# GadGadGad/Convolutional-KAN-for-Image-Classification

Hardware: AMD Instinct MI355X
Metric: images/sec fwd+bwd KAN-VGG11 3x32x32 bs=256/GPU (higher is better)
Workload: dtype f32

## Files before the change

### convolutional-kan-for-image-classification_amd/_lib.py

```python
from __future__ import annotations

import ctypes as C
import os
from typing import Optional

_HERE = os.path.dirname(os.path.abspath(__file__))
LIB_PATH = os.environ.get("KANCONV_LIB") or os.path.join(_HERE, "libkanconv.so")

KAN_MAX_PLANES = 16
KAN_MAX_TABLE = 32
KAN_FP_WORDS = 192
BASIS_BSPLINE, BASIS_RBF, BASIS_CHEBY, BASIS_POLY, BASIS_FOURIER, BASIS_RELU, BASIS_GRAM = 0, 1, 2, 3, 4, 5, 6
ACT_NONE, ACT_IDENTITY, ACT_GELU, ACT_SILU, ACT_RELU, ACT_TANH, ACT_SIGMOID, ACT_GELU_TANH = -1, 0, 1, 2, 3, 4, 5, 6


class KanGeom(C.Structure):
    _fields_ = [(n, C.c_int) for n in ("B", "C", "H", "W", "O", "Ho", "Wo", "kh", "kw", "sh", "sw", "ph", "pw", "dh", "dw", "groups")] + \
               [("x_bstride", C.c_longlong), ("y_bstride", C.c_longlong)]


class KanBasis(C.Structure):
    _fields_ = [("kind", C.c_int), ("n_basis", C.c_int), ("order", C.c_int), ("act", C.c_int),
                ("p0", C.c_float), ("p1", C.c_float), ("table", C.c_float * KAN_MAX_TABLE), ("chan_table", C.c_void_p)]


class KanPlan(C.Structure):
    _fields_ = [(n, C.c_int) for n in ("P", "K", "IPC", "KC", "Kpad", "Opad", "fwd_splits", "bwd_data_splits", "bwd_weight_splits",
                                          "fwd_target", "bwd_data_target", "bwd_weight_target", "x_pm_wanted", "dz_pm_wanted", "bwd_weight_expanded", "row_blocks", "e_pm_wanted", "fwd_expanded", "fwd_halo", "bwd_weight_halo",
                                          "fwd_band", "bwd_weight_band")] + \
               [(n, C.c_longlong) for n in ("packed_weight_bytes", "bwd_data_weight_bytes", "fwd_slab_elems", "bwd_data_slab_elems",
                                            "bwd_weight_slab_elems", "e_pm_elems")]


class KanWavGeom(C.Structure):
    _fields_ = [(n, C.c_int) for n in ("B", "C", "H", "W", "O", "Ho", "Wo", "kh", "kw", "sh", "sw", "ph", "pw", "dh", "dw", "wavelet")] + \
               [("x_bstride", C.c_longlong), ("u_bstride", C.c_longlong)]


WAVELETS = {"mexican_hat": 0, "morlet": 1, "dog": 2, "meyer": 3, "shannon": 4}

_P, _I, _LL, _F, _D = C.c_void_p, C.c_int, C.c_longlong, C.c_float, C.c_double
_GP, _BP = C.POINTER(KanGeom), C.POINTER(KanBasis)
SIGNATURES = {
    "kan_version": (C.c_char_p, []),
    "kan_last_error": (C.c_char_p, []),
    "kan_plan": (_I, [_GP, _BP, C.POINTER(KanPlan)]),
    "kan_pack_weights": (_I, [_P, _P, _P, _P, _GP, _BP, _P]),
    "kan_pack_cacheable": (_I, [_GP, _BP]),
    "kan_pack_weights_cached": (_I, [_P, _P, _P, _P, _GP, _BP, _P, _I, _I, _I, _P]),
    "kan_conv_fwd": (_I, [_P, _P, _P, _P, _GP, _BP, _P, _P]),
    "kan_position_major": (_I, [_P, _P, _I, _I, _I, _LL, _P]),
    "kan_conv_bwd_data": (_I, [_P, _P, _P, _P, _P, _P, _GP, _BP, _P, _P]),
    "kan_conv_bwd_data_params": (_I, [_P, _P, _P, _P, _P, _P, _P, _GP, _BP, _P, _P]),
    "kan_conv_bwd_weight": (_I, [_P, _P, _P, _P, _GP, _BP, _P, _P, _P]),
    "kan_position_major_expanded": (_I, [_P, _P, _GP, _BP, _P]),
    "kan_conv_fwd_expanded": (_I, [_P, _P, _P, _GP, _BP, _P]),
    "kan_conv_bwd_weight_expanded": (_I, [_P, _P, _P, _GP, _BP, _P]),
    "kan_unpack_wgrad": (_I, [_P, _P, _P, _GP, _BP, _P]),
    "kan_slab_reduce": (_I, [_P, _I, _LL, _P, _I, _I, _I, _LL, _P]),
    "kan_instnorm_prelu_fwd": (_I, [_P, _I, _LL, _P, _P, _P, _P, _P, _P, _P, _I, _I, _I, _LL, _F, _I, _P]),
    "kan_instnorm_prelu_bwd": (_I, [_P, _P, _P, _P, _P, _P, _P, _P, _P, _P, _P, _I, _I, _I, _LL, _I, _P]),
    "kan_instnorm_prelu_pool_fwd": (_I, [_P, _I, _LL, _P, _P, _P, _P, _P, _P, _P, _P, _I, _I, _I, _I, _LL, _F, _I, _P]),
    "kan_instnorm_prelu_pool_bwd": (_I, [_P, _P, _P, _P, _P, _P, _P, _P, _P, _P, _P, _P, _I, _I, _I, _I, _LL, _I, _P]),
    "kan_instnorm_prelu_poolk_fwd": (_I, [_P, _I, _LL, _P, _P, _P, _P, _P, _P, _P, _P, _I, _I, _I, _I, _LL, _F, _I, _I, _I, _P]),
    "kan_instnorm_prelu_poolk_bwd": (_I, [_P, _P, _P, _P, _P, _P, _P, _P, _P, _P, _P, _P, _I, _I, _I, _I, _LL, _I, _I, _I, _P]),
    "kan_split_supported": (_I, [C.POINTER(KanGeom), C.POINTER(KanBasis)]),
    "kan_split_weight_bytes": (_LL, [C.POINTER(KanGeom), C.POINTER(KanBasis)]),
    "kan_split_pack_weights": (_I, [_P, _P, _P, C.POINTER(KanGeom), C.POINTER(KanBasis), _P]),
    "kan_conv_fwd_split": (_I, [_P, _P, _P, C.POINTER(KanGeom), C.POINTER(KanBasis), _P]),
# ... 39 lines not shown
```

### convolutional-kan-for-image-classification_amd/csrc/kan_internal.h

```cpp
#pragma once
#include <type_traits>
#include "kanconv.h"

int kan_fail_msg(const char* fmt, const char* a);
int kan_raise_lds_limit(const void* kernel, int bytes);

enum : int {
    FAST_GENERIC = 0,
    FAST_BSPLINE_SILU = 1,
    FAST_BSPLINE_GELU = 2,
    FAST_RBF8 = 3,
    FAST_CHEBY5 = 4,
    FAST_CHEBY4 = 5,
    FAST_POLY4 = 6,
    FAST_POLY3 = 7,
    FAST_RBF5 = 8,
    FAST_RELU8 = 9,
    FAST_GRAM4 = 10,
    FAST_POLY1 = 11,
    FAST_LAST = 11
};
enum : unsigned {
    ON_TAP_MAJOR = 1u << 0,
    ON_BIG_TILES = 1u << 1,
    ON_HALO_FWD = 1u << 2,
    ON_HALO_BWD_WEIGHT = 1u << 3,
    ON_BAND_FWD = 1u << 4,
    ON_BAND_BWD_WEIGHT = 1u << 5,
    ON_EXPANDED_FWD = 1u << 6,
    ON_EXPANDED = 1u << 7,
    ON_ROWBLK_BWD_DATA = 1u << 8,
};
struct FastSpec {
    int kind, planes;
    bool base;
    bool xn_fwd, xn_bwd;
    int kc;
    unsigned routes;
};
constexpr FastSpec fast_spec(int f) {
    constexpr unsigned bspline = ON_TAP_MAJOR | ON_BIG_TILES | ON_HALO_FWD | ON_HALO_BWD_WEIGHT | ON_BAND_FWD | ON_BAND_BWD_WEIGHT |
                                 ON_EXPANDED_FWD | ON_EXPANDED | ON_ROWBLK_BWD_DATA;
    switch (f) {
        case FAST_BSPLINE_SILU: case FAST_BSPLINE_GELU: return {KAN_BASIS_BSPLINE, 9, true, false, false, 18, bspline};
        case FAST_RBF8: return {KAN_BASIS_RBF, 9, true, true, true, 18, ON_TAP_MAJOR | ON_BAND_FWD | ON_BAND_BWD_WEIGHT};
        case FAST_RBF5: return {KAN_BASIS_RBF, 6, true, true, true, 18, ON_TAP_MAJOR};
        case FAST_CHEBY5: return {KAN_BASIS_CHEBY, 5, false, false, false, 16, ON_TAP_MAJOR | ON_BIG_TILES | ON_BAND_FWD | ON_BAND_BWD_WEIGHT};
        case FAST_CHEBY4: return {KAN_BASIS_CHEBY, 4, false, false, false, 16, ON_TAP_MAJOR | ON_HALO_FWD | ON_BAND_FWD};
        case FAST_POLY4: return {KAN_BASIS_POLY, 5, true, true, false, 16, ON_TAP_MAJOR | ON_BIG_TILES | ON_HALO_FWD | ON_BAND_FWD};
        case FAST_POLY3: return {KAN_BASIS_POLY, 4, true, true, false, 16, ON_TAP_MAJOR};
        case FAST_POLY1: return {KAN_BASIS_POLY, 2, true, true, false, 16, ON_TAP_MAJOR};
        case FAST_RELU8: return {KAN_BASIS_RELU, 9, true, false, false, 16, ON_HALO_FWD | ON_HALO_BWD_WEIGHT | ON_EXPANDED_FWD | ON_EXPANDED};
        case FAST_GRAM4: return {KAN_BASIS_GRAM, 5, true, false, false, 16, ON_HALO_FWD | ON_HALO_BWD_WEIGHT | ON_EXPANDED};
        default: return {-1, 0, false, true, true, 0, 0};
    }
}
constexpr int fast_kind(int f) { return fast_spec(f).kind; }
constexpr int fast_planes(int f) { return fast_spec(f).planes; }
constexpr bool fast_has(int f, unsigned routes) { return (fast_spec(f).routes & routes) == routes && f != FAST_GENERIC; }

template <int V> using IC = std::integral_constant<int, V>;
template <unsigned ROUTES, int F = 1, class Fn>
bool dispatch_fast(int f, Fn&& fn) {
    if constexpr (F > FAST_LAST) {
        return false;
// ... 28 lines not shown
    int cells;
    int slots;
    int TS;
    int lds_bytes, wgs_per_cu;
    int fwd_splits;
    int bw_ok, bw_WR, bw_NI, bw_NT, bw_tiles_o, bw_row_tiles, bw_TPI, bw_ptiles, bw_cells, bw_slots, bw_lds_bytes, bw_splits;
    unsigned short bw_ph_rt0[KAN_BAND_MAX_PHASES + 1];
    unsigned char ph_a[KAN_BAND_MAX_PHASES], ph_b[KAN_BAND_MAX_PHASES];
    short ph_tap0[KAN_BAND_MAX_PHASES + 1];
    unsigned short tap_shift[KAN_BAND_MAX_TAPS];
    unsigned short tap_rt[KAN_BAND_MAX_TAPS];
    short tap_step[KAN_BAND_MAX_TAPS], tap_nt[KAN_BAND_MAX_TAPS];
} KanBandCfg;

void kan_band_cfg(const KanGeom* g, const KanBasis* b, int fast, KanBandCfg* cfg);
int kan_band_bwd_weight_launch(const float* dz, const float* x, const float* xn, float* dwp, const KanGeom* g, const KanBasis* b,
                               const KanBandCfg* cfg, int splits, long long slab_elems, void* stream);
int kan_band_fwd_launch(const float* x, const float* xn, const float* wp, float* z, const KanGeom* g, const KanBasis* b,
                        const KanBandCfg* cfg, int splits, long long slab_elems, void* stream);

constexpr int DW_T = 9;
constexpr int DW_MAX_TP = 96;

enum class Route { TAP_MAJOR, DW, BAND, HALO, EXPANDED };

struct FwdCfg { int TO, TP, tiles_o, tiles_p, chunks, splits, slots; };
struct BdCfg { int CH, tiles_c, tiles_p, n_ob, Opad32, chunks, splits; };
struct BwCfg { int TR, TO, tiles_r, tiles_o, chunks, splits, slots; };
struct BwHaloCfg { int R, nimg, spb, n_bands, tiles_r, tiles_o, splits, bands_per_split; };

struct ConvPlan {
    KanPlan pub;
    int fast;
    Route fwd, bwd_data, bwd_weight;
    bool pm_fwd, pm_bwd_data, pm_bwd_weight;
    bool rowblk_bwd_data;
    bool pmdma_xcd, pm_lpt, pm_xcd;
    FwdCfg fc;
    BdCfg bd;
    BwCfg bw;
    BwHaloCfg bwh;
    KanBandCfg band;
};
int plan_conv(const KanGeom* g, const KanBasis* b, ConvPlan* cp);

int live_taps_out(const KanGeom* g, int hw);
int live_taps_in(const KanGeom* g, int hw);
// ... 3 lines not shown
```

### convolutional-kan-for-image-classification_amd/csrc/kan_plan.hip

```cpp
#include <hip/hip_runtime.h>
#include <cstdio>
#include <cstdlib>
#include <cstring>
#include "kanconv.h"
#include "kan_device.h"
#include "kan_common.h"
#include "kan_internal.h"

namespace {

int fail(const char* msg) { return kan_fail_msg("%s", msg); }

int check(const KanGeom* g, const KanBasis* b) {
    if (!g || !b) return fail("null geometry/basis");
    if (g->groups < 0 || g->groups > 65535) return fail("groups out of range");
    if (g->B <= 0 || g->C <= 0 || g->O <= 0 || g->H <= 0 || g->W <= 0 || g->Ho <= 0 || g->Wo <= 0) return fail("non-positive dimension");
    if (g->kh <= 0 || g->kw <= 0 || g->sh <= 0 || g->sw <= 0 || g->dh <= 0 || g->dw <= 0 || g->ph < 0 || g->pw < 0) return fail("bad conv parameters");
    if (g->kh > 255 || g->kw > 255 || g->C > 65535) return fail("kernel size / channel count out of supported range");
    if ((g->H + 2 * g->ph - g->dh * (g->kh - 1) - 1) / g->sh + 1 != g->Ho || (g->W + 2 * g->pw - g->dw * (g->kw - 1) - 1) / g->sw + 1 != g->Wo)
        return fail("Ho/Wo inconsistent with H/W, kernel, stride, padding, dilation");
    if ((long long)g->B * g->Ho * g->Wo >= (1ll << 31) || (long long)g->B * g->H * g->W >= (1ll << 31)) return fail("pixel count exceeds int32");
    if ((long long)g->B * g->x_bstride * 4 >= (1ll << 31) || (long long)g->B * g->y_bstride * 4 >= (1ll << 31))
        return fail("activation tensors must be smaller than 2 GiB (32-bit buffer offsets)");
    if (g->x_bstride < (long long)ngroups(g) * g->C * g->H * g->W || g->y_bstride < (long long)ngroups(g) * g->O * g->Ho * g->Wo)
// ... 124 lines not shown
    return !tuning_off("KAN_BD_ROWBLK") && fast_has(f, ON_ROWBLK_BWD_DATA) && !pm_bwd_data && g->H == 4 && g->W == 4 && g->Ho == 4 && g->Wo == 4 &&
           g->kh == 3 && g->kw == 3 && g->sh == 1 && g->sw == 1 && g->ph == 1 && g->pw == 1 && g->dh == 1 && g->dw == 1 && g->B % 8 == 0 && g->O % 16 == 0;
}
struct LiveClass { long long tiles; int live_steps; };

int pick_target_steps(const LiveClass* cls, int ncls, int min_steps, double slab_bytes, int* max_splits, long long SLOTS = 1024) {
    int hi = 1;
    for (int i = 0; i < ncls; ++i) if (cls[i].live_steps > hi) hi = cls[i].live_steps;
    int best = hi; double best_cost = -1; int best_ms = 1;
    for (int t = min_steps < hi ? min_steps : hi; t <= hi; ++t) {
        long long wgs = 0; int ms = 1;
        for (int i = 0; i < ncls; ++i) {
            const int sp = cls[i].live_steps > 0 ? ceil_div(cls[i].live_steps, t) : 1;
            wgs += cls[i].tiles * sp;
            if (sp > ms) ms = sp;
        }
        const long long rounds = (wgs + SLOTS - 1) / SLOTS;
        const double cost = (double)(rounds * (t + 6)) + ms * slab_cost_steps(slab_bytes);
        if (best_cost < 0 || cost < best_cost) { best_cost = cost; best = t; best_ms = ms; }
    }
    *max_splits = best_ms;
    return best;
}
BdCfg bd_cfg(const KanGeom* g, const KanPlan& pl) {
    BdCfg c;
    c.CH = 64 / pl.P;
    c.tiles_c = ceil_div(g->C, 2 * c.CH);
    c.tiles_p = ceil_div((long long)g->B * g->H * g->W, 128);
    c.n_ob = ceil_div(g->O, 16);
    c.Opad32 = round_up(g->O, 32);
    c.chunks = g->kh * g->kw * c.n_ob;
    c.splits = pick_splits((long long)c.tiles_c * c.tiles_p * ngroups(g), c.chunks, 8, 4.0 * g->B * g->C * g->H * g->W * ngroups(g));
    return c;
}
bool pmdma_bwd_weight(const KanGeom* g, const KanBasis* b, int f, bool want_pm_bw) {
    if (tuning_off("KAN_PMDMA") || !fast_has(f, ON_EXPANDED)) return false;
    if (!want_pm_bw) return false;
    const int P = b->n_basis + (b->act != KAN_ACT_NONE);
    return (g->C * P) % 128 == 0 && g->B % 16 == 0 && round_up(g->O, 64) % 128 == 0 &&
           (long long)g->C * g->H * g->W * P * g->B * 4 < (1ll << 31);
}
bool halo_bwd_weight(const KanGeom* g, int f, bool pmdma_bw) {
    if (tuning_off("KAN_HALO_BW") || !fast_has(f, ON_HALO_BWD_WEIGHT)) return false;
    if (g->kh != 3 || g->kw != 3 || g->sh != 1 || g->sw != 1 || g->dh != 1 || g->dw != 1 || g->ph != 1 || g->pw != 1) return false;
    if (round_up(g->O, 64) % 128 != 0 || g->C > 65535 / 81) return false;
    if (g->H != g->W) return false;
// ... 102 lines not shown
    if (int rc = check(g, b)) return rc;
    ConvPlan& c = *cp;
    KanPlan* pl = &c.pub;
    const int T = g->kh * g->kw, G = ngroups(g), f = fast_variant(b);
    c.fast = f;
    const bool pm_shape = pmdma_fwd_shape(g, f);
    c.pm_fwd = want_pix_major(g, b, PM_FWD, pm_shape);
    c.pm_bwd_data = want_pix_major(g, b, PM_BWD_DATA, false);
    const bool want_pm_bw = want_pix_major(g, b, PM_BWD_WEIGHT, false);
    const bool dw = dw_direct(g, b);
    const bool halo = halo_fwd(g, b, f, c.pm_fwd);
    c.band.ok = c.band.bw_ok = 0;
    const bool band = band_fwd(g, b, f, dw, c.pm_fwd, halo, &c.band);
    const bool pmdma_fwd = pm_shape && c.pm_fwd;
    const bool pmdma_bw = pmdma_bwd_weight(g, b, f, want_pm_bw);
    const bool halo_bw = halo_bwd_weight(g, f, pmdma_bw);
    c.pm_bwd_weight = want_pm_bw && !halo_bw;
    const bool band_bw = band && c.band.bw_ok && !want_pm_bw && !tuning_off("KAN_BAND_BW");
    c.rowblk_bwd_data = rowblk_bwd_data(g, f, c.pm_bwd_data);
    c.pmdma_xcd = tuning_on("KAN_PMDMA_XCD");
    c.pm_lpt = !tuning_off("KAN_PM_LPT");
    c.pm_xcd = !tuning_off("KAN_PM_XCD");
    c.fwd = dw ? Route::DW : band ? Route::BAND : halo ? Route::HALO : pmdma_fwd ? Route::EXPANDED : Route::TAP_MAJOR;
    c.bwd_data = dw ? Route::DW : Route::TAP_MAJOR;
    c.bwd_weight = dw ? Route::DW : band_bw ? Route::BAND : halo_bw ? Route::HALO : pmdma_bw ? Route::EXPANDED : Route::TAP_MAJOR;
    pl->P = b->n_basis + (b->act != KAN_ACT_NONE);
    pl->K = g->C * T * pl->P;
    {
        int i18 = 18 / pl->P, i16 = 16 / pl->P;
        if (i18 > 4) i18 = 4;
        if (i16 > 4) i16 = 4;
        const bool use18 = (long long)i18 * pl->P * 16 > (long long)i16 * pl->P * 18;
        pl->KC = use18 ? 18 : 16;
        pl->IPC = use18 ? i18 : i16;
        if (pl->P >= 10 && pl->P <= 12) { pl->KC = 12; pl->IPC = 1; }
        if (halo) { pl->KC = 2 * pl->P; pl->IPC = 2; }
    }
    pl->Kpad = ceil_div(g->C * T, pl->IPC) * pl->KC;
    if (band) { pl->KC = c.band.NPLE; pl->IPC = c.band.NG; pl->Kpad = c.band.n_steps * c.band.NPLE; }
    pl->Opad = round_up(g->O, 64);
    pl->packed_weight_bytes = (long long)G * pl->Kpad * pl->Opad * 4;
    c.bd = bd_cfg(g, *pl);
    pl->bwd_data_weight_bytes = (long long)G * T * c.bd.Opad32 * c.bd.tiles_c * 128 * 4;
    pl->fwd_slab_elems = (long long)g->B * g->y_bstride;
    pl->bwd_data_slab_elems = (long long)g->B * g->x_bstride;
    pl->bwd_weight_slab_elems = (long long)G * pl->K * pl->Opad;
    const bool big = big_tiles(f, *pl);
// ... 50 lines not shown
```

### convolutional-kan-for-image-classification_amd/csrc/kanconv.hip

```cpp
#include <hip/hip_runtime.h>
#include <cstdio>
#include <cstdlib>
#include <cstring>
#include <cmath>
#include <cstdint>
#include <mutex>
#include <type_traits>
#include <vector>
#include "kanconv.h"
#include "kan_device.h"

#include "kan_common.h"
#include "kan_internal.h"

namespace {


thread_local char g_err[512] = "";
int fail(const char* fmt, const char* a = "") {
    snprintf(g_err, sizeof(g_err), fmt, a);
    return -1;
}
}
int kan_fail_msg(const char* fmt, const char* a) { return fail(fmt, a); }
// ... 567 lines not shown
    int base = 0;
    int m = M;
#pragma unroll
    for (int off = 32; off >= 1; off >>= 1) {
        if (m > 1) {
            const int h = m / 2;
            const bool up = (lane & off) != 0;
#pragma unroll
            for (int i = 0; i < M / 2; ++i) {
                if (i < h) {
                    const float keep = up ? v[h + i] : v[i], send = up ? v[i] : v[h + i];
                    v[i] = keep + __shfl_xor(send, off, 64);
                }
            }
            base += up ? h : 0;
            m = h;
        } else {
            v[0] += __shfl_xor(v[0], off, 64);
        }
    }
    idx = base; tot = v[0];
}

template <int KIND, int FAST, int RB = 0>
__global__ __launch_bounds__(256, 4) void k_conv_bwd_data(
    const float* __restrict__ dz, const float* __restrict__ x, const float* __restrict__ xn, const float* __restrict__ wd,
    float* __restrict__ dx, float* __restrict__ dxn, DevGeom g, DevBasis bs, int CH, int n_ct, int n_ob, int Opad16,
    int n_chunks, int chunks_per_split, long long slab_elems, unsigned dz_bytes, TilePerm perm, float* __restrict__ dpar) {
    constexpr int TP = 128, KD = 16, NT = 256;
    __shared__ __attribute__((aligned(16))) float smem[2 * 2 * KD * 128];
    __shared__ float sTab[KAN_MAX_TABLE];

    const int tid = threadIdx.x, lane = tid & 63;
    const int wave = __builtin_amdgcn_readfirstlane(tid >> 6);
    const int w_r = wave >> 1, w_p = wave & 1;
    const int HoWo = g.Ho * g.Wo, HW = g.H * g.W, P = bs.P;
    const int Min = g.B * HW;
    const BlockId blk = xcd_block_order(false);
    const int grp = blk.y / n_ct;
    const int px_tile0 = (perm.n ? (int)perm.idx[blk.x] : blk.x) * TP, ct = blk.y - grp * n_ct;
    const int ncol = n_ct * 128;
    const int pxl = (wave & 1) * 64 + lane, ol0 = wave >> 1;
    const bool idle_rows = (ct * 2 + w_r) * CH >= g.C;
    {
        const size_t xo = (size_t)grp * g.C * HW;
        x += xo; xn += xo; dx += xo; if (dxn) dxn += xo;
// ... 135 lines not shown
    };
    int ch = next_live(ch0);
    if (ch < ch1) { if (RB) issue_rb(ch, 0); else issue(ch, 0); }
    const int ar = w_r * 64 + (lane & 31), bp = w_p * 64 + (lane & 31), kh2 = lane >> 5;
    for (int cur = 0; ch < ch1; cur ^= 1) {
        asm volatile("s_waitcnt vmcnt(0)" ::: "memory");
        __syncthreads();
        const bool mixed_now = pend_mixed;
        ch = next_live(ch + 1);
        if (ch < ch1) { if (RB) issue_rb(ch, cur ^ 1); else issue(ch, cur ^ 1); }
        const float* cW = smem + cur * (2 * KD * 128);
        const float* cG = cW + KD * 128;
        const unsigned aw = lds_addr(cW + kh2 * 128 + ar), ag = lds_addr(cG + kh2 * TP + bp);
        if (RB) {
            const bool l0b = !(mixed_now && w_p == 0), l1a = !(mixed_now && w_p == 1);
            if (!idle_rows) KAN_MFMA_STEP_LIVE(KD / 2, aw, 128, ag, TP, true, l0b, l1a, true);
        } else if (!idle_rows) KAN_MFMA_STEP(KD / 2, aw, 128, ag, TP);
    }

    const bool same_in = (x == xn);
    const bool split_out = (dxn != nullptr);
    float* dxs = dx + (size_t)blk.z * slab_elems;
    float* dxns = split_out ? dxn + (size_t)blk.z * slab_elems : nullptr;
#define KAN_G_TO_LDS(half)                                                                                                 \
    __syncthreads();                                                                                                       \
    if (w_r == (half)) {                                                                                                   \
        _Pragma("unroll") for (int mi = 0; mi < 2; ++mi)                                                                   \
            _Pragma("unroll") for (int ni = 0; ni < 2; ++ni)                                                               \
                _Pragma("unroll") for (int r = 0; r < 16; ++r)                                                             \
                    smem[(mi * 32 + mfma_row(r, lane)) * TP + w_p * 64 + ni * 32 + (lane & 31)] = acc[mi][ni][r];          \
    }                                                                                                                      \
    __syncthreads();
    if constexpr (FAST != 0) {
        constexpr FastSpec S = fast_spec(FAST);
        constexpr int FP = S.planes, FCH = 64 / FP, NIT = (FCH + 1) / 2, NPF = S.xn_bwd ? 1 : 2;
        float xv[NPF][NIT], nv[NIT]; unsigned ok = 0;
#define KAN_FETCH(half, slot)                                                                                              \
        _Pragma("unroll") for (int it = 0; it < NIT; ++it) {                                                                   \
            const int cl = ol0 + 2 * it, c = (ct * 2 + (half)) * FCH + cl;                                                     \
            const bool v = cl < FCH && c < g.C && pv;                                                                          \
            const size_t idx = (size_t)pb * g.xbs + (size_t)c * HW + (size_t)(ph_ * g.W + pw_);                                \
            xv[slot][it] = v ? x[idx] : 0.f;                                                                                   \
            if constexpr (S.xn_bwd) nv[it] = v ? xn[idx] : 0.f;                                                                \
            ok |= (v ? 1u : 0u) << ((slot) * NIT + it);                                                                        \
        }
        if constexpr (!S.xn_bwd) {
#pragma unroll
            for (int half = 0; half < 2; ++half) KAN_FETCH(half, half)
        }
#pragma unroll 1
        for (int half = 0; half < 2; ++half) {
            if constexpr (S.xn_bwd) { ok = 0; KAN_FETCH(half, 0) }
            KAN_G_TO_LDS(half)
#pragma unroll
            for (int it = 0; it < NIT; ++it) {
                if (!((ok >> ((S.xn_bwd ? 0 : half) * NIT + it)) & 1u)) continue;
                const int cl = ol0 + 2 * it, c = (ct * 2 + half) * FCH + cl;
                const float xa = (S.xn_bwd || half == 0) ? xv[0][it] : xv[NPF - 1][it];
                const InGrad d = stage_unit_grad<KIND, FAST>(bs, sTab, xa, S.xn_bwd ? nv[it] : xa, smem + (cl * FP) * TP + pxl, TP);
                const size_t idx = (size_t)pb * g.xbs + (size_t)c * HW + (size_t)(ph_ * g.W + pw_);
                dxs[idx] = d.dx;
                if constexpr (S.xn_bwd) dxns[idx] = d.dxn;
            }
        }
#undef KAN_FETCH
        return;
    }
#pragma unroll 1
    for (int half = 0; half < 2; ++half) {
        KAN_G_TO_LDS(half)
#undef KAN_G_TO_LDS
        for (int cl = ol0; cl < CH; cl += 2) {
            const int c = (ct * 2 + half) * CH + cl;
            if (c >= g.C || !pv) continue;
            const size_t idx = (size_t)pb * g.xbs + (size_t)c * HW + (size_t)(ph_ * g.W + pw_);
            const float xa = x[idx];
            const float xb = same_in ? xa : xn[idx];
            float s_base = 0.f, s_bas = 0.f;
            const float* Gc = smem + (cl * P) * TP + pxl;
            kan_planes_each<KIND, true>(bs, sTab, xa, xb, c, [&](int p, float d) {
                const float gv = Gc[p * TP];
                if (p < bs.hb) s_base += d * gv; else s_bas += d * gv;
            });
            if (split_out) { dxs[idx] = s_base; dxns[idx] = s_bas; }
            else dxs[idx] = s_base + s_bas;
        }
        if (KIND == KAN_BASIS_GRAM && dpar) {
            const int nb = bs.nb;
            const unsigned slot = (blockIdx.x + 7u * blockIdx.y + 13u * blockIdx.z) & 63u;
#pragma unroll 1
            for (int m = 1; m < nb - 1; ++m) {
                DevBasis bm = bs; bm.order = m;
                float am = 0.f;
                for (int cl = ol0; cl < CH; cl += 2) {
// ... 28 lines not shown
                            vlo = -(q2 * x2) * gv; vhi = (q2 * x1) * gv;
                        }
                        v[j] = vlo; v[8 + j] = vhi;
                    }
                    int idx; float tot;
                    wave_reduce_scatter<16>(v, lane, idx, tot);
                    const int j = idx & 7;
                    if ((lane & 3) == 0 && j < nb) atomicAdd(dpar + (size_t)c * 2 * nb + (idx < 8 ? j : nb + j), tot);
                } else {
                    for (int j = 0; j < nb; ++j) {
                        const float gv = pv ? smem[(cl * P + hb + j) * TP + pxl] : 0.f;
                        const float x1 = fmaxf(xb - lo[j], 0.f), x2 = fmaxf(lo[nb + j] - xb, 0.f);
                        const float q2 = 2.0f * (x1 * x2 * rr) * rr;
                        float vlo = -(q2 * x2) * gv, vhi = (q2 * x1) * gv;
#pragma unroll
                        for (int off = 32; off > 0; off >>= 1) { vlo += __shfl_xor(vlo, off, 64); vhi += __shfl_xor(vhi, off, 64); }
                        if (lane == 0) { atomicAdd(dpar + (size_t)c * 2 * nb + j, vlo); atomicAdd(dpar + (size_t)c * 2 * nb + nb + j, vhi); }
                    }
                }
            }
        }
    }
}

template <int KIND, int FAST, int WR, int WC>
__global__ __launch_bounds__(WR * WC * 64, (WR * WC > 4 ? 2 : 4)) void k_conv_bwd_weight(
    const float* __restrict__ dz, const float* __restrict__ x, const float* __restrict__ xn, float* __restrict__ dwp,
    DevGeom g, DevBasis bs, int Krows, int Opad, int n_chunks, int chunks_per_split, long long slab_elems,
    unsigned x_bytes, unsigned dz_bytes, int tiles_o) {
    constexpr int TR = WR * 64, TO = WC * 64, NT = WR * WC * 64, KPX = 16;
    constexpr int MRG = KAN_PMAX;
    constexpr int LDE = TR + 2 * MRG + 1, LDZ = TO + 1;
    constexpr int IPP = NT / KPX;
    constexpr int UPF = TR / 128;
    constexpr int ZL = TO * KPX / NT;
    constexpr int MAXI = TR + 2;
    __shared__ float sE[2 * KPX * LDE];
    __shared__ float sZ[2 * KPX * LDZ];
    __shared__ int sItem[MAXI];
    __shared__ float sTab[KAN_MAX_TABLE];
    __shared__ float sDump[NT];

    const int tid = threadIdx.x, lane = tid & 63;
    const int wave = __builtin_amdgcn_readfirstlane(tid >> 6);
    const int w_r = wave / WC, w_c = wave % WC;
    const int HoWo = g.Ho * g.Wo, HW = g.H * g.W, T = g.kh * g.kw, P = FAST ? fast_planes(FAST) : bs.P;
// ... 1332 lines not shown
    a.decay = (float)(1.0 - lr * weight_decay);
    a.w1 = (float)(1.0 - beta1); a.b2 = (float)beta2; a.w2 = (float)(1.0 - beta2);
    a.gscale = grad_scale; a.inv_bc2_sqrt = (float)(1.0 / sqrt(bc2)); a.eps = (float)eps; a.neg_step = (float)(-lr / bc1);
    return a;
}

#include "wavkan.inc"

}

extern "C" {

const char* kan_version(void) { return "kanconv 0.5 (gfx950, fp32 MFMA 32x32x2, halo forward, 128/256-output tiles)"; }
const char* kan_last_error(void) { return g_err; }

int kan_plan(const KanGeom* geom, const KanBasis* basis, KanPlan* plan) {
    if (!plan) return fail("null plan");
    ConvPlan cp;
    if (int rc = plan_conv(geom, basis, &cp)) return rc;
    *plan = cp.pub;
    return 0;
}

static bool pack_needs_clear(const KanGeom* g, const KanPlan& pl) {
    if (pl.fwd_band) return pl.KC != pl.IPC * pl.P || g->C % pl.IPC != 0;
    return pl.KC != pl.IPC * pl.P || (g->C * g->kh * g->kw) % pl.IPC != 0;
}

static int pack_weights_impl(const float* w_base, const float* w_basis, float* wp, float* wd, const KanGeom* g, const KanBasis* b,
                             const unsigned long long* fp, int fp_cur, void* stream) {
    ConvPlan cp;
    if (int rc = plan_conv(g, b, &cp)) return rc;
    const KanPlan& pl = cp.pub;
    const int hb = b->act != KAN_ACT_NONE;
    if ((hb && !w_base) || !w_basis || !wp) return fail("null weight pointer");
    hipStream_t st = (hipStream_t)stream;
    const int T = g->kh * g->kw, NI = g->C * T, G = ngroups(g);
    const long long wp_gs = (long long)pl.Kpad * pl.Opad;
    PackGeo q = pack_geo(g, b, cp, false);
    if (fp && (pack_needs_clear(g, pl) || cp.fwd == Route::DW)) return fail("cached packing is not offered for this geometry (kan_pack_cacheable)");
    if (pl.KC != pl.IPC * pl.P || (pl.fwd_band && pack_needs_clear(g, pl))) {
        if (hipMemsetAsync(wp, 0, (size_t)pl.packed_weight_bytes, st) != hipSuccess) return fail("memset failed");
    } else if (!pl.fwd_band && NI % pl.IPC != 0) {
        if (G > 1) {
            if (hipMemsetAsync(wp, 0, (size_t)pl.packed_weight_bytes, st) != hipSuccess) return fail("memset failed");
        } else {
// ... 190 lines not shown
        DevGeom dgd = dev_geom(g); DevBasis dbd = dev_basis(b);
        dim3 grid(ceil_div((long long)g->B * g->H * g->W, 256), ngroups(g));
        dispatch_kind(b->kind, [&](auto kind) {
            hipLaunchKernelGGL((k_dw_bwd_data<decltype(kind)::value>), grid, dim3(256), 0, st, dz, x, xn, wd, dx, dxn, dgd, dbd, pl.Opad, pl.IPC, pl.KC, pl.Kpad);
        });
        return launch_ok("dw_bwd_data");
    }
    const BdCfg& c = cp.bd;
    DevGeom dg = dev_geom(g);
    dg.pix_major = (dz_pm && cp.pm_bwd_data) ? 1 : 0;
    if (dg.pix_major) dz = dz_pm;
    DevBasis db = dev_basis(b);
    if ((long long)c.tiles_c * ngroups(g) > 65535) return fail("groups * channel tiles exceed the grid limit");
    dim3 grid(c.tiles_p, c.tiles_c * ngroups(g), pl.bwd_data_splits);
    const int cps = dg.pix_major ? pl.bwd_data_target : ceil_div(c.chunks, pl.bwd_data_splits);
    TilePerm perm; perm.n = 0;
    if (dg.pix_major) perm = tile_perm(c.tiles_p, [&](int t) {
        const int hw = (int)(((long long)t * 128) / g->B);
        return ceil_div(live_taps_in(g, hw < g->H * g->W ? hw : 0) * c.n_ob, cps > 0 ? cps : 1);
    });
    const int fast = (fast_spec(cp.fast).xn_bwd ? (x != xn && dxn) : (x == xn && !dxn)) ? cp.fast : FAST_GENERIC;
    const bool rb = !dg.pix_major && cp.rowblk_bwd_data;
    const unsigned dz_bytes = (unsigned)((long long)g->B * g->y_bstride * 4);
    auto launch = [&](auto kind, auto fast, auto rbv) {
        hipLaunchKernelGGL((k_conv_bwd_data<decltype(kind)::value, decltype(fast)::value, decltype(rbv)::value>), grid, dim3(256), 0, st, dz, x, xn, wd,
                           dx, dxn, dg, db, c.CH, c.tiles_c, c.n_ob, c.Opad32, c.chunks, cps, pl.bwd_data_slab_elems, dz_bytes, perm, dpar);
    };
    const bool launched = dispatch_fast<ON_TAP_MAJOR>(fast, [&](auto fv) {
        constexpr int F = decltype(fv)::value;
        if constexpr (fast_has(F, ON_ROWBLK_BWD_DATA)) {
            if (rb) return launch(IC<fast_kind(F)>{}, fv, IC<1>{});
        }
        launch(IC<fast_kind(F)>{}, fv, IC<0>{});
    });
    if (!launched) dispatch_kind(b->kind, [&](auto kind) { launch(kind, IC<FAST_GENERIC>{}, IC<0>{}); });
    return launch_ok("conv_bwd_data");
}

int kan_conv_bwd_weight(const float* dz, const float* x, const float* xn, float* dwp, const KanGeom* g, const KanBasis* b,
                        const float* x_pm, const float* dz_pm, void* stream) {
    ConvPlan cp;
    if (int rc = plan_conv(g, b, &cp)) return rc;
    const KanPlan& pl = cp.pub;
    if (!dz || !x || !xn || !dwp) return fail("null tensor pointer");
    if ((b->kind == KAN_BASIS_RELU || b->kind == KAN_BASIS_GRAM) && !b->chan_table) return fail("ReLU / Gram bases need their device parameter table (chan_table)");
    hipStream_t st = (hipStream_t)stream;
// ... 308 lines not shown
```

### include/kanconv.h

```cpp
#ifndef KANCONV_H
#define KANCONV_H

#ifdef __cplusplus
extern "C" {
#endif

#define KAN_MAX_PLANES 16
#define KAN_MAX_TABLE  32
#define KAN_FP_WORDS   192

enum { KAN_BASIS_BSPLINE = 0, KAN_BASIS_RBF = 1, KAN_BASIS_CHEBY = 2, KAN_BASIS_POLY = 3, KAN_BASIS_FOURIER = 4, KAN_BASIS_RELU = 5, KAN_BASIS_GRAM = 6 };
enum { KAN_ACT_NONE = -1, KAN_ACT_IDENTITY = 0, KAN_ACT_GELU = 1, KAN_ACT_SILU = 2, KAN_ACT_RELU = 3,
       KAN_ACT_TANH = 4, KAN_ACT_SIGMOID = 5, KAN_ACT_GELU_TANH = 6 };

typedef struct KanGeom {
    int B, C, H, W;
    int O, Ho, Wo;
    int kh, kw, sh, sw, ph, pw, dh, dw;
    int groups;
    long long x_bstride;
    long long y_bstride;
} KanGeom;

typedef struct KanBasis {
// ... 10 lines not shown
    int Kpad, Opad;
    int fwd_splits;
    int bwd_data_splits;
    int bwd_weight_splits;
    int fwd_target, bwd_data_target, bwd_weight_target;
    int x_pm_wanted, dz_pm_wanted;
    int bwd_weight_expanded;
    int row_blocks;
    int e_pm_wanted, fwd_expanded;
    int fwd_halo, bwd_weight_halo;
    int fwd_band, bwd_weight_band;
    long long packed_weight_bytes;
    long long bwd_data_weight_bytes;
    long long fwd_slab_elems;
    long long bwd_data_slab_elems;
    long long bwd_weight_slab_elems;
    long long e_pm_elems;
} KanPlan;

const char* kan_version(void);
const char* kan_last_error(void);

int kan_plan(const KanGeom* geom, const KanBasis* basis, KanPlan* plan);

int kan_pack_weights(const float* w_base, const float* w_basis, float* wp, float* wd,
                     const KanGeom* geom, const KanBasis* basis, void* stream);

int kan_pack_cacheable(const KanGeom* geom, const KanBasis* basis);
int kan_pack_weights_cached(const float* w_base, const float* w_basis, float* wp, float* wd,
                            const KanGeom* geom, const KanBasis* basis, unsigned long long* ring, int cur, int force,
                            int sample_stride, void* stream);

int kan_conv_fwd(const float* x, const float* xn, const float* wp, float* z,
                 const KanGeom* geom, const KanBasis* basis, const float* x_pm, void* stream);

int kan_position_major(const float* src, float* dst, int B, int Cn, int HW, long long bstride, void* stream);

int kan_conv_bwd_data(const float* dz, const float* x, const float* xn, const float* wd,
                      float* dx, float* dxn,
                      const KanGeom* geom, const KanBasis* basis, const float* dz_pm, void* stream);

int kan_conv_bwd_data_params(const float* dz, const float* x, const float* xn, const float* wd, float* dx, float* dxn, float* dparams,
                             const KanGeom* geom, const KanBasis* basis, const float* dz_pm, void* stream);

int kan_conv_bwd_weight(const float* dz, const float* x, const float* xn, float* dwp,
                        const KanGeom* geom, const KanBasis* basis, const float* x_pm, const float* dz_pm, void* stream);
// ... 70 lines not shown
```

Baseline: 17270.

## Add halo-tiled backward-data kernel for 3x3 stride-1 KAN convs on small maps

Adds a new backward-data kernel that stages dz tiles with a halo in LDS and reuses them across all nine taps, instead of gathering tap-major expanded data. The route is selected for B-spline 3x3 stride-1 pad-1 layers. By default only the 4x4 row-block case uses it; wider maps need an opt-in flag. The fast epilogue is factored into macros so both kernels share it. The goal is less redundant global traffic on dz in the late VGG layers. The cost is extra kernel complexity and tap-split MFMA masking.

```diff
diff --git a/convolutional-kan-for-image-classification_amd/_lib.py b/convolutional-kan-for-image-classification_amd/_lib.py
--- a/convolutional-kan-for-image-classification_amd/_lib.py
+++ b/convolutional-kan-for-image-classification_amd/_lib.py
@@ -37,6 +37,9 @@
                [("x_bstride", C.c_longlong), ("u_bstride", C.c_longlong)]
 
 
+STAGE_FWD, STAGE_BWD_DATA, STAGE_BWD_WEIGHT = 0, 1, 2
+ROUTE_TAP_MAJOR, ROUTE_DW, ROUTE_BAND, ROUTE_HALO, ROUTE_EXPANDED = 0, 1, 2, 3, 4
+
 WAVELETS = {"mexican_hat": 0, "morlet": 1, "dog": 2, "meyer": 3, "shannon": 4}
 
 _P, _I, _LL, _F, _D = C.c_void_p, C.c_int, C.c_longlong, C.c_float, C.c_double
@@ -45,6 +48,7 @@
     "kan_version": (C.c_char_p, []),
     "kan_last_error": (C.c_char_p, []),
     "kan_plan": (_I, [_GP, _BP, C.POINTER(KanPlan)]),
+    "kan_stage_route": (_I, [_GP, _BP, _I]),
     "kan_pack_weights": (_I, [_P, _P, _P, _P, _GP, _BP, _P]),
     "kan_pack_cacheable": (_I, [_GP, _BP]),
     "kan_pack_weights_cached": (_I, [_P, _P, _P, _P, _GP, _BP, _P, _I, _I, _I, _P]),
diff --git a/convolutional-kan-for-image-classification_amd/csrc/kan_internal.h b/convolutional-kan-for-image-classification_amd/csrc/kan_internal.h
--- a/convolutional-kan-for-image-classification_amd/csrc/kan_internal.h
+++ b/convolutional-kan-for-image-classification_amd/csrc/kan_internal.h
@@ -30,6 +30,7 @@
     ON_EXPANDED_FWD = 1u << 6,
     ON_EXPANDED = 1u << 7,
     ON_ROWBLK_BWD_DATA = 1u << 8,
+    ON_HALO_BWD_DATA = 1u << 9,
 };
 struct FastSpec {
     int kind, planes;
@@ -40,7 +41,7 @@
 };
 constexpr FastSpec fast_spec(int f) {
     constexpr unsigned bspline = ON_TAP_MAJOR | ON_BIG_TILES | ON_HALO_FWD | ON_HALO_BWD_WEIGHT | ON_BAND_FWD | ON_BAND_BWD_WEIGHT |
-                                 ON_EXPANDED_FWD | ON_EXPANDED | ON_ROWBLK_BWD_DATA;
+                                 ON_EXPANDED_FWD | ON_EXPANDED | ON_ROWBLK_BWD_DATA | ON_HALO_BWD_DATA;
     switch (f) {
         case FAST_BSPLINE_SILU: case FAST_BSPLINE_GELU: return {KAN_BASIS_BSPLINE, 9, true, false, false, 18, bspline};
         case FAST_RBF8: return {KAN_BASIS_RBF, 9, true, true, true, 18, ON_TAP_MAJOR | ON_BAND_FWD | ON_BAND_BWD_WEIGHT};
@@ -115,7 +116,7 @@
 constexpr int DW_T = 9;
 constexpr int DW_MAX_TP = 96;
 
-enum class Route { TAP_MAJOR, DW, BAND, HALO, EXPANDED };
+enum class Route { TAP_MAJOR = KAN_ROUTE_TAP_MAJOR, DW = KAN_ROUTE_DW, BAND = KAN_ROUTE_BAND, HALO = KAN_ROUTE_HALO, EXPANDED = KAN_ROUTE_EXPANDED };
 
 struct FwdCfg { int TO, TP, tiles_o, tiles_p, chunks, splits, slots; };
 struct BdCfg { int CH, tiles_c, tiles_p, n_ob, Opad32, chunks, splits; };
diff --git a/convolutional-kan-for-image-classification_amd/csrc/kan_plan.hip b/convolutional-kan-for-image-classification_amd/csrc/kan_plan.hip
--- a/convolutional-kan-for-image-classification_amd/csrc/kan_plan.hip
+++ b/convolutional-kan-for-image-classification_amd/csrc/kan_plan.hip
@@ -170,6 +170,14 @@
     *max_splits = best_ms;
     return best;
 }
+bool halo_bwd_data(const KanGeom* g, int f, bool pm_bwd_data, bool rowblk) {
+    if (tuning_off("KAN_BD_HALO") || !fast_has(f, ON_HALO_BWD_DATA)) return false;
+    if (g->kh != 3 || g->kw != 3 || g->sh != 1 || g->sw != 1 || g->dh != 1 || g->dw != 1 || g->ph != 1 || g->pw != 1) return false;
+    if (pm_bwd_data || ngroups(g) != 1 || g->O % 16 != 0) return false;
+    const int W = g->W, H = g->H;
+    if (W == 4 && H == 4) return rowblk;
+    return tuning_on("KAN_BD_HALO_WIDE") && ((W == 16 && H % 8 == 0) || (W == 8 && H == 8));
+}
 BdCfg bd_cfg(const KanGeom* g, const KanPlan& pl) {
     BdCfg c;
     c.CH = 64 / pl.P;
@@ -318,7 +326,7 @@
     c.pm_lpt = !tuning_off("KAN_PM_LPT");
     c.pm_xcd = !tuning_off("KAN_PM_XCD");
     c.fwd = dw ? Route::DW : band ? Route::BAND : halo ? Route::HALO : pmdma_fwd ? Route::EXPANDED : Route::TAP_MAJOR;
-    c.bwd_data = dw ? Route::DW : Route::TAP_MAJOR;
+    c.bwd_data = dw ? Route::DW : halo_bwd_data(g, f, c.pm_bwd_data, c.rowblk_bwd_data) ? Route::HALO : Route::TAP_MAJOR;
     c.bwd_weight = dw ? Route::DW : band_bw ? Route::BAND : halo_bw ? Route::HALO : pmdma_bw ? Route::EXPANDED : Route::TAP_MAJOR;
     pl->P = b->n_basis + (b->act != KAN_ACT_NONE);
     pl->K = g->C * T * pl->P;
diff --git a/convolutional-kan-for-image-classification_amd/csrc/kanconv.hip b/convolutional-kan-for-image-classification_amd/csrc/kanconv.hip
--- a/convolutional-kan-for-image-classification_amd/csrc/kanconv.hip
+++ b/convolutional-kan-for-image-classification_amd/csrc/kanconv.hip
@@ -613,6 +613,45 @@
     idx = base; tot = v[0];
 }
 
+#define KAN_G_TO_LDS(half)                                                                                                 \
+    __syncthreads();                                                                                                       \
+    if (w_r == (half)) {                                                                                                   \
+        _Pragma("unroll") for (int mi = 0; mi < 2; ++mi)                                                                   \
+            _Pragma("unroll") for (int ni = 0; ni < 2; ++ni)                                                               \
+                _Pragma("unroll") for (int r = 0; r < 16; ++r)                                                             \
+                    smem[(mi * 32 + mfma_row(r, lane)) * TP + w_p * 64 + ni * 32 + (lane & 31)] = acc[mi][ni][r];          \
+    }                                                                                                                      \
+    __syncthreads();
+#define KAN_FETCH(half, slot)                                                                                              \
+        _Pragma("unroll") for (int it = 0; it < NIT; ++it) {                                                                   \
+            const int cl = ol0 + 2 * it, c = (ct * 2 + (half)) * FCH + cl;                                                     \
+            const bool v = cl < FCH && c < g.C && pv;                                                                          \
+            const size_t idx = (size_t)pb * g.xbs + (size_t)c * HW + (size_t)(ph_ * g.W + pw_);                                \
+            xv[slot][it] = v ? x[idx] : 0.f;                                                                                   \
+            if constexpr (S.xn_bwd) nv[it] = v ? xn[idx] : 0.f;                                                                \
+            ok |= (v ? 1u : 0u) << ((slot) * NIT + it);                                                                        \
+        }
+#define KAN_BD_FAST_EPILOGUE()                                                                                             \
+        constexpr FastSpec S = fast_spec(FAST);                                                                            \
+        constexpr int FP = S.planes, FCH = 64 / FP, NIT = (FCH + 1) / 2, NPF = S.xn_bwd ? 1 : 2;                           \
+        float xv[NPF][NIT], nv[NIT]; unsigned ok = 0;                                                                      \
+        if constexpr (!S.xn_bwd) {                                                                                         \
+            _Pragma("unroll") for (int half = 0; half < 2; ++half) KAN_FETCH(half, half)                                   \
+        }                                                                                                                  \
+        _Pragma("unroll 1") for (int half = 0; half < 2; ++half) {                                                         \
+            if constexpr (S.xn_bwd) { ok = 0; KAN_FETCH(half, 0) }                                                         \
+            KAN_G_TO_LDS(half)                                                                                             \
+            _Pragma("unroll") for (int it = 0; it < NIT; ++it) {                                                           \
+                if (!((ok >> ((S.xn_bwd ? 0 : half) * NIT + it)) & 1u)) continue;                                          \
+                const int cl = ol0 + 2 * it, c = (ct * 2 + half) * FCH + cl;                                               \
+                const float xa = (S.xn_bwd || half == 0) ? xv[0][it] : xv[NPF - 1][it];                                    \
+                const InGrad d = stage_unit_grad<KIND, FAST>(bs, sTab, xa, S.xn_bwd ? nv[it] : xa, smem + (cl * FP) * TP + pxl, TP); \
+                const size_t idx = (size_t)pb * g.xbs + (size_t)c * HW + (size_t)(ph_ * g.W + pw_);                        \
+                dxs[idx] = d.dx;                                                                                           \
+                if constexpr (S.xn_bwd) dxns[idx] = d.dxn;                                                                 \
+            }                                                                                                              \
+        }                                                                                                                  \
+        return;
 template <int KIND, int FAST, int RB = 0>
 __global__ __launch_bounds__(256, 4) void k_conv_bwd_data(
     const float* __restrict__ dz, const float* __restrict__ x, const float* __restrict__ xn, const float* __restrict__ wd,
@@ -794,54 +833,10 @@
     const bool split_out = (dxn != nullptr);
     float* dxs = dx + (size_t)blk.z * slab_elems;
     float* dxns = split_out ? dxn + (size_t)blk.z * slab_elems : nullptr;
-#define KAN_G_TO_LDS(half)                                                                                                 \
-    __syncthreads();                                                                                                       \
-    if (w_r == (half)) {                                                                                                   \
-        _Pragma("unroll") for (int mi = 0; mi < 2; ++mi)                                                                   \
-            _Pragma("unroll") for (int ni = 0; ni < 2; ++ni)                                                               \
-                _Pragma("unroll") for (int r = 0; r < 16; ++r)                                                             \
-                    smem[(mi * 32 + mfma_row(r, lane)) * TP + w_p * 64 + ni * 32 + (lane & 31)] = acc[mi][ni][r];          \
-    }                                                                                                                      \
-    __syncthreads();
-    if constexpr (FAST != 0) {
-        constexpr FastSpec S = fast_spec(FAST);
-        constexpr int FP = S.planes, FCH = 64 / FP, NIT = (FCH + 1) / 2, NPF = S.xn_bwd ? 1 : 2;
-        float xv[NPF][NIT], nv[NIT]; unsigned ok = 0;
-#define KAN_FETCH(half, slot)                                                                                              \
-        _Pragma("unroll") for (int it = 0; it < NIT; ++it) {                                                                   \
-            const int cl = ol0 + 2 * it, c = (ct * 2 + (half)) * FCH + cl;                                                     \
-            const bool v = cl < FCH && c < g.C && pv;                                                                          \
-            const size_t idx = (size_t)pb * g.xbs + (size_t)c * HW + (size_t)(ph_ * g.W + pw_);                                \
-            xv[slot][it] = v ? x[idx] : 0.f;                                                                                   \
-            if constexpr (S.xn_bwd) nv[it] = v ? xn[idx] : 0.f;                                                                \
-            ok |= (v ? 1u : 0u) << ((slot) * NIT + it);                                                                        \
-        }
-        if constexpr (!S.xn_bwd) {
-#pragma unroll
-            for (int half = 0; half < 2; ++half) KAN_FETCH(half, half)
-        }
-#pragma unroll 1
-        for (int half = 0; half < 2; ++half) {
-            if constexpr (S.xn_bwd) { ok = 0; KAN_FETCH(half, 0) }
-            KAN_G_TO_LDS(half)
-#pragma unroll
-            for (int it = 0; it < NIT; ++it) {
-                if (!((ok >> ((S.xn_bwd ? 0 : half) * NIT + it)) & 1u)) continue;
-                const int cl = ol0 + 2 * it, c = (ct * 2 + half) * FCH + cl;
-                const float xa = (S.xn_bwd || half == 0) ? xv[0][it] : xv[NPF - 1][it];
-                const InGrad d = stage_unit_grad<KIND, FAST>(bs, sTab, xa, S.xn_bwd ? nv[it] : xa, smem + (cl * FP) * TP + pxl, TP);
-                const size_t idx = (size_t)pb * g.xbs + (size_t)c * HW + (size_t)(ph_ * g.W + pw_);
-                dxs[idx] = d.dx;
-                if constexpr (S.xn_bwd) dxns[idx] = d.dxn;
-            }
-        }
-#undef KAN_FETCH
-        return;
-    }
+    if constexpr (FAST != 0) { KAN_BD_FAST_EPILOGUE() }
 #pragma unroll 1
     for (int half = 0; half < 2; ++half) {
         KAN_G_TO_LDS(half)
-#undef KAN_G_TO_LDS
         for (int cl = ol0; cl < CH; cl += 2) {
             const int c = (ct * 2 + half) * CH + cl;
             if (c >= g.C || !pv) continue;
@@ -916,6 +911,163 @@
         }
     }
 }
+
+#define KAN_MFMA_STEP_HALO(addrA, addrB1, addrB2, OPB, QB, l0a, l0b, l1a, l1b)                                                       \
+    do {                                                                                                                           \
+        float fa_[2][2], fb_[2][2];                                                                                                \
+        LDS_READ4(fa_[0][0], fa_[0][1], fb_[0][0], fb_[0][1], addrA, addrB1, 0, 32 * 4, 0, (QB));                                  \
+        _Pragma("unroll") for (int kk = 0; kk < 8; ++kk) {                                                                          \
+            const int c_ = kk & 1, n_ = c_ ^ 1;                                                                                    \
+            if (kk + 1 < 4) {                                                                                                      \
+                LDS_READ4(fa_[n_][0], fa_[n_][1], fb_[n_][0], fb_[n_][1], addrA, addrB1, (2 * (kk + 1)) * 128 * 4,                 \
+                          (2 * (kk + 1)) * 128 * 4 + 128, (2 * (kk + 1)) * (OPB), (2 * (kk + 1)) * (OPB) + (QB));                  \
+                LDS_WAIT4(fa_[c_][0], fa_[c_][1], fb_[c_][0], fb_[c_][1], 4);                                                      \
+            } else if (kk + 1 < 8) {                                                                                               \
+                LDS_READ4(fa_[n_][0], fa_[n_][1], fb_[n_][0], fb_[n_][1], addrA, addrB2, (2 * (kk + 1)) * 128 * 4,                 \
+                          (2 * (kk + 1)) * 128 * 4 + 128, (2 * ((kk + 1) & 3)) * (OPB), (2 * ((kk + 1) & 3)) * (OPB) + (QB));      \
+                LDS_WAIT4(fa_[c_][0], fa_[c_][1], fb_[c_][0], fb_[c_][1], 4);                                                      \
+            } else {                                                                                                               \
+                LDS_WAIT4(fa_[c_][0], fa_[c_][1], fb_[c_][0], fb_[c_][1], 0);                                                      \
+            }                                                                                                                      \
+            if (kk < 4 ? (l0a) : (l0b)) {                                                                                          \
+                acc[0][0] = MFMA32(fa_[c_][0], fb_[c_][0], acc[0][0]);                                                             \
+                acc[1][0] = MFMA32(fa_[c_][1], fb_[c_][0], acc[1][0]);                                                             \
+            }                                                                                                                      \
+            if (kk < 4 ? (l1a) : (l1b)) {                                                                                          \
+                acc[0][1] = MFMA32(fa_[c_][0], fb_[c_][1], acc[0][1]);                                                             \
+                acc[1][1] = MFMA32(fa_[c_][1], fb_[c_][1], acc[1][1]);                                                             \
+            }                                                                                                                      \
+        }                                                                                                                          \
+    } while (0)
+
+template <int FAST, int W, int R, int NIMG>
+__global__ __launch_bounds__(256, 4) void k_conv_bwd_data_halo(
+    const float* __restrict__ dz, const float* __restrict__ x, const float* __restrict__ wd, float* __restrict__ dx, DevGeom g, DevBasis bs,
+    int n_ct, int n_ob, int Opad16, long long slab_elems, unsigned dz_bytes) {
+    constexpr int KIND = fast_kind(FAST), TP = 128, KD = 16, NT = 256, NSTEP = 9;
+    constexpr int HW_ = W == 16 ? 20 : W + 2, HIMG = NIMG == 2 ? 112 : (R + 2) * HW_, HALO = NIMG * HIMG;
+    constexpr int OP = (HALO + 15) / 32 * 32 + 16;
+    constexpr bool ROWBLK = (R * W == 16);
+    constexpr int SROWS = NIMG == 1 ? R + 2 : R, NSRC = NIMG * SROWS * W, CPT = NSRC / 16;
+    constexpr int QOFF = HW_;
+    constexpr int SMEM = 2 * KD * 128 + KD * OP > 64 * TP ? 2 * KD * 128 + KD * OP : 64 * TP;
+    static_assert(NIMG * R * W == TP && NSRC % 16 == 0 && OP >= HALO && HIMG >= (R + 2) * HW_, "tile shape");
+    __shared__ __attribute__((aligned(16))) float smem[SMEM];
+    __shared__ float sTab[KAN_MAX_TABLE];
+    float* const sW = smem;
+    float* const sH = smem + 2 * KD * 128;
+
+    const int tid = threadIdx.x, lane = tid & 63;
+    const int wave = __builtin_amdgcn_readfirstlane(tid >> 6);
+    const int w_r = wave >> 1, w_p = wave & 1;
+    const int HW = g.H * W, Min = g.B * HW;
+    const BlockId blk = xcd_block_order(false);
+    const int px_tile0 = blk.x * TP, ct = blk.y;
+    const int ncol = n_ct * 128;
+    const int pxl = w_p * 64 + lane, ol0 = w_r;
+    const bool idle_rows = (ct * 2 + w_r) * (64 / fast_planes(FAST)) >= g.C;
+    const float* xn = x; float* dxns = nullptr;
+
+    if (tid < KAN_MAX_TABLE) sTab[tid] = bs.tab[tid];
+    for (int i = tid; i < KD * OP; i += NT) sH[i] = 0.f;
+    const int my_px = px_tile0 + (ROWBLK      ? ((pxl >> 2) & 7) * 16 + (pxl >> 5) * 4 + (pxl & 3)
+                                  : NIMG == 1 ? ((pxl >> 5) + 4 * ((pxl >> 4) & 1)) * 16 + (pxl & 15)
+                                              : ((pxl >> 4) & 1) * 64 + ((pxl >> 5) + 4 * ((pxl >> 3) & 1)) * 8 + (pxl & 7));
+    const bool pv = my_px < Min;
+    const int pb = my_px / HW, ph_ = (my_px - pb * HW) / W, pw_ = (my_px - pb * HW) % W;
+
+    const int b0 = px_tile0 / HW, h0 = (px_tile0 - b0 * HW) / W;
+    const kan_rsrc dz_rs = make_rsrc(dz, dz_bytes);
+    const int sj = tid & 15, so = tid >> 4;
+    const unsigned vsrc = (unsigned)(so * HW + sj) * 4u;
+    float* const vdst = sH + so * OP + (NIMG == 1 ? sj + 1 : ROWBLK ? ((sj >> 2) + 1) * HW_ + (sj & 3) + 1 : ((sj >> 3) + 1) * HW_ + (sj & 7) + 1);
+    unsigned s_ok = 0; int s_off[CPT];
+#pragma unroll
+    for (int k = 0; k < CPT; ++k) {
+        const int img = NIMG == 1 ? 0 : ROWBLK ? k : k >> 2;
+        const bool ok = NIMG == 1 ? (unsigned)(h0 - 1 + k) < (unsigned)g.H : b0 + img < g.B;
+        s_ok |= (ok ? 1u : 0u) << k;
+        s_off[k] = (b0 + img) * (int)g.ybs + (NIMG == 1 ? (h0 - 1 + k) * W : ROWBLK ? 0 : (k & 3) * 16);
+    }
+    constexpr auto dst_off = [](int k) { return NIMG == 1 ? k * HW_ : ROWBLK ? k * HIMG : (k >> 2) * HIMG + (k & 3) * 2 * HW_; };
+    float zv[CPT];
+    auto load_block = [&](int ob) {
+#pragma unroll
+        for (int k = 0; k < CPT; ++k)
+            if ((s_ok >> k) & 1u)
+                zv[k] = __builtin_bit_cast(float, __builtin_amdgcn_raw_buffer_load_b32(dz_rs, (int)vsrc, (s_off[k] + ob * KD * HW) * 4, 0));
+    };
+
+    const int kh2 = lane >> 5, l31 = lane & 31;
+    const int cell = NIMG == 1 ? (2 * w_p + 4 * (l31 >> 4) + 1) * HW_ + (l31 & 15) + 1
+                   : ROWBLK    ? (l31 >> 2) * HIMG + (2 * w_p + 1) * HW_ + (l31 & 3) + 1
+                               : (l31 >> 4) * HIMG + (2 * w_p + 4 * ((l31 >> 3) & 1) + 1) * HW_ + (l31 & 7) + 1;
+    const unsigned vb = lds_addr(sH + kh2 * OP + cell);
+    const int ar = w_r * 64 + l31;
+    const unsigned wlane = (unsigned)((lane >> 5) * ncol + (lane & 31) * 4) * 4u;
+    const int wv = wave;
+
+    struct Step { int tapA, tapB, oA, oB; };
+    auto decode = [&](int u) -> Step {
+        if (ROWBLK && u >= 3) { const int t = (u - 3) >> 1, hf = (u - 3) & 1; return {t, 6 + t, 8 * hf, 8 * hf}; }
+        const int tap = ROWBLK ? 3 + u : u;
+        return {tap, tap, 0, 8};
+    };
+    auto issue_w = [&](int ob, int u, int buf) {
+        const Step s = decode(u);
+        float* dW = sW + buf * (KD * 128);
+#pragma unroll
+        for (int j = 0; j < 2; ++j) {
+            const int blk2 = j * 4 + wv;
+            const int row = (blk2 < 4 ? s.tapA * Opad16 + s.oA : s.tapB * Opad16 + s.oB) + ob * KD + (blk2 & 3) * 2;
+            glds16((const float*)((const char*)(wd + (size_t)row * ncol + ct * 128) + wlane), dW + blk2 * 256);
+        }
+    };
+
+    f32x16 acc[2][2];
+#pragma unroll
+    for (int a = 0; a < 2; ++a)
+#pragma unroll
+        for (int b = 0; b < 2; ++b)
+#pragma unroll
+            for (int r = 0; r < 16; ++r) acc[a][b][r] = 0.f;
+
+    const int n_steps = n_ob * NSTEP;
+    const int s0 = (int)((long long)n_steps * blk.z / gridDim.z), s1 = (int)((long long)n_steps * (blk.z + 1) / gridDim.z);
+    int ob = s0 / NSTEP, u = s0 - ob * NSTEP, pref = ob, buf = 0;
+    if (s0 < s1) { issue_w(ob, u, 0); load_block(ob); }
+    bool fresh = true;
+#pragma unroll 1
+    for (int s = s0; s < s1; ++s) {
+        if (fresh) {
+            __syncthreads();
+#pragma unroll
+            for (int k = 0; k < CPT; ++k)
+                if ((s_ok >> k) & 1u) vdst[dst_off(k)] = zv[k];
+            fresh = false;
+        }
+        asm volatile("s_waitcnt vmcnt(0)" ::: "memory");
+        __syncthreads();
+        const int un = u + 1 == NSTEP ? 0 : u + 1, obn = u + 1 == NSTEP ? ob + 1 : ob;
+        if (s + 1 < s1) issue_w(obn, un, buf ^ 1);
+        if (u >= NSTEP / 2 && pref == ob && (ob + 1) * NSTEP < s1) { load_block(ob + 1); pref = ob + 1; }
+        const Step st = decode(u);
+        const int shA = (1 - st.tapA / 3) * HW_ + (1 - st.tapA % 3), shB = (1 - st.tapB / 3) * HW_ + (1 - st.tapB % 3);
+        const unsigned aw = lds_addr(sW + buf * (KD * 128) + kh2 * 128 + ar);
+        const unsigned abA = vb + (unsigned)((st.oA * OP + shA) * 4), abB = vb + (unsigned)((st.oB * OP + shB) * 4);
+        if (ROWBLK) {
+            const bool mixed = u >= 3;
+            const bool l0b = !(mixed && w_p == 0), l1a = !(mixed && w_p == 1);
+            if (!idle_rows) KAN_MFMA_STEP_HALO(aw, abA, abB, OP * 4, QOFF * 4, true, l0b, l1a, true);
+        } else if (!idle_rows) KAN_MFMA_STEP_HALO(aw, abA, abB, OP * 4, QOFF * 4, true, true, true, true);
+        buf ^= 1; u = un; fresh = obn != ob; ob = obn;
+    }
+
+    float* dxs = dx + (size_t)blk.z * slab_elems;
+    KAN_BD_FAST_EPILOGUE()
+}
+#undef KAN_FETCH
+#undef KAN_G_TO_LDS
 
 template <int KIND, int FAST, int WR, int WC>
 __global__ __launch_bounds__(WR * WC * 64, (WR * WC > 4 ? 2 : 4)) void k_conv_bwd_weight(
@@ -2294,6 +2446,17 @@
     return 0;
 }
 
+int kan_stage_route(const KanGeom* geom, const KanBasis* basis, int stage) {
+    ConvPlan cp;
+    if (int rc = plan_conv(geom, basis, &cp)) return rc;
+    switch (stage) {
+        case KAN_STAGE_FWD: return (int)cp.fwd;
+        case KAN_STAGE_BWD_DATA: return (int)cp.bwd_data;
+        case KAN_STAGE_BWD_WEIGHT: return (int)cp.bwd_weight;
+        default: return fail("kan_stage_route: unknown stage");
+    }
+}
+
 static bool pack_needs_clear(const KanGeom* g, const KanPlan& pl) {
     if (pl.fwd_band) return pl.KC != pl.IPC * pl.P || g->C % pl.IPC != 0;
     return pl.KC != pl.IPC * pl.P || (g->C * g->kh * g->kw) % pl.IPC != 0;
@@ -2530,6 +2693,18 @@
     const int fast = (fast_spec(cp.fast).xn_bwd ? (x != xn && dxn) : (x == xn && !dxn)) ? cp.fast : FAST_GENERIC;
     const bool rb = !dg.pix_major && cp.rowblk_bwd_data;
     const unsigned dz_bytes = (unsigned)((long long)g->B * g->y_bstride * 4);
+    if (cp.bwd_data == Route::HALO && fast != FAST_GENERIC && !dpar && !dg.pix_major) {
+        dispatch_fast<ON_HALO_BWD_DATA>(fast, [&](auto fv) {
+            auto launch_halo = [&](auto w, auto r, auto nimg) {
+                hipLaunchKernelGGL((k_conv_bwd_data_halo<decltype(fv)::value, decltype(w)::value, decltype(r)::value, decltype(nimg)::value>), grid,
+                                   dim3(256), 0, st, dz, x, wd, dx, dg, db, c.tiles_c, c.n_ob, c.Opad32, pl.bwd_data_slab_elems, dz_bytes);
+            };
+            if (g->W == 16) launch_halo(IC<16>{}, IC<8>{}, IC<1>{});
+            else if (g->W == 8) launch_halo(IC<8>{}, IC<8>{}, IC<2>{});
+            else launch_halo(IC<4>{}, IC<4>{}, IC<8>{});
+        });
+        return launch_ok("conv_bwd_data_halo");
+    }
     auto launch = [&](auto kind, auto fast, auto rbv) {
         hipLaunchKernelGGL((k_conv_bwd_data<decltype(kind)::value, decltype(fast)::value, decltype(rbv)::value>), grid, dim3(256), 0, st, dz, x, xn, wd,
                            dx, dxn, dg, db, c.CH, c.tiles_c, c.n_ob, c.Opad32, c.chunks, cps, pl.bwd_data_slab_elems, dz_bytes, perm, dpar);
diff --git a/include/kanconv.h b/include/kanconv.h
--- a/include/kanconv.h
+++ b/include/kanconv.h
@@ -56,6 +56,10 @@
 const char* kan_last_error(void);
 
 int kan_plan(const KanGeom* geom, const KanBasis* basis, KanPlan* plan);
+
+enum { KAN_STAGE_FWD = 0, KAN_STAGE_BWD_DATA = 1, KAN_STAGE_BWD_WEIGHT = 2 };
+enum { KAN_ROUTE_TAP_MAJOR = 0, KAN_ROUTE_DW = 1, KAN_ROUTE_BAND = 2, KAN_ROUTE_HALO = 3, KAN_ROUTE_EXPANDED = 4 };
+int kan_stage_route(const KanGeom* geom, const KanBasis* basis, int stage);
 
 int kan_pack_weights(const float* w_base, const float* w_basis, float* wp, float* wd,
                      const KanGeom* geom, const KanBasis* basis, void* stream);
```

After: 17300, median of 6. About the same (+0.2%).
